# stone-d-chen/ffvvc

Measured on AMD Instinct MI355X. Metric: decoded frames/sec (4K/8K 10-bit VVC) per GPU, higher is better.
Workload: dtype u16

## Files before the change

ffvvc_amd/csrc/itx.hip:

```cpp
#include <type_traits>
#include "common.hpp"
#include "pk16.hpp"
#include "wave.hpp"
#include "runtime.hpp"
#include "resid_math.hpp"
#include "../../include/vvc_mi355.h"
#include "stage_checks.hpp"

namespace vvc355 {

#define VVC355_TABLE(type, name, count) __device__ static const type d_tab_##name[count]
#include "tables.inc"
#undef VVC355_TABLE
#define VVC355_TABLE(type, name, count) static constexpr type c_##name[count]
#include "tables_small.inc"
#undef VVC355_TABLE
__host__ __device__ constexpr int level_scale_of(int rect, int rem)
{
    return rect ? (rem == 0 ? 57 : rem == 1 ? 64 : rem == 2 ? 72 : rem == 3 ? 80 : rem == 4 ? 90 : 102)
                : (rem == 0 ? 40 : rem == 1 ? 45 : rem == 2 ? 51 : rem == 3 ? 57 : rem == 4 ? 64 : 72);
}
static constexpr unsigned long long kDiag4X = 0x3323213210210100ull, kDiag4Y = 0x3231230123012010ull;
constexpr bool itx_small_tables_match()
{
    for (int r = 0; r < 2; r++)
        for (int q = 0; q < 6; q++)
            if (level_scale_of(r, q) != c_level_scale[r * 6 + q]) return false;
    for (int i = 0; i < 16; i++)
        if ((int)((kDiag4X >> (4 * i)) & 15) != c_diag_scan_4x4_x[i] || (int)((kDiag4Y >> (4 * i)) & 15) != c_diag_scan_4x4_y[i]) return false;
    return true;
}
static_assert(itx_small_tables_match(), "level scale / 4x4 diagonal scan differ from vvc_intra.c:329-336 / vvc_data.c:27,152");

enum { TX_DCT2 = 0, TX_DST7 = 1, TX_DCT8 = 2 };

__device__ __forceinline__ const int8_t *dxt_matrix(int type, int n)
{
    if (type == TX_DST7)
        return n == 4 ? d_tab_dst7_4 : n == 8 ? d_tab_dst7_8 : n == 16 ? d_tab_dst7_16 : d_tab_dst7_32;
    return n == 4 ? d_tab_dct8_4 : n == 8 ? d_tab_dct8_8 : n == 16 ? d_tab_dct8_16 : d_tab_dct8_32;
}

__device__ __forceinline__ int inputs_used(int type, int n, int nz)
{
    if (type != TX_DCT2)
        return nz;
    int used = 2;
    while (used < nz)
        used <<= 1;
    used = min(used, n);
    return n == 64 ? min(used, 32) : used;
}

__device__ __forceinline__ int inv_tx_out(int type, int n, int i, const int *in, int step, int cnt, const int8_t *cos_lds)
{
    unsigned acc = 0;
    if (type == TX_DCT2) {
        const int ang = (2 * i + 1) * (64 / n);
        for (int k = 0; k < cnt; k++)
            acc += (unsigned)in[k * step] * (unsigned)(int)cos_lds[(ang * k) & 255];
    } else {
        const int8_t *m = dxt_matrix(type, n) + i;
        for (int k = 0; k < cnt; k++)
            acc += (unsigned)in[k * step] * (unsigned)(int)m[k * n];
    }
    return (int)acc;
}

__host__ __device__ inline int derive_tr_type(int flags, int mts_idx, int lfnst_idx, int c_idx, int w, int h)
{
    const bool isp = flags & VVC355_TU_ISP, sbt = flags & VVC355_TU_SBT;
    if (c_idx || (isp && lfnst_idx))
        return 0;
    bool implicit = false;
    if (flags & VVC355_TU_MTS_ENABLED)
        implicit = isp || (sbt && (w > h ? w : h) <= 32) ||
                   (!(flags & VVC355_TU_EXPLICIT_MTS_INTRA) && (flags & VVC355_TU_INTRA) && !lfnst_idx && !(flags & VVC355_TU_MIP));
    if (implicit) {
        int trh, trv;
        if (sbt) {
            const bool hor = flags & VVC355_TU_SBT_HORIZONTAL, pos = flags & VVC355_TU_SBT_POS;
            trh = (hor || pos) ? 1 : 2;
            trv = (!hor || pos) ? 1 : 2;
        } else {
            trh = (w >= 4 && w <= 16) ? 1 : 0;
            trv = (h >= 4 && h <= 16) ? 1 : 0;
        }
        return trh | (trv << 4);
    }
    const int trh = mts_idx == 0 ? 0 : (mts_idx & 1) ? 1 : 2, trv = mts_idx == 0 ? 0 : mts_idx <= 2 ? 1 : 2;
    return trh | (trv << 4);
}
__device__ __forceinline__ void resolve_type(vvc355_itx_job &job)
{
    if (job.mts_flags & VVC355_ITX_DERIVE_TYPE) {
        const int t = derive_tr_type(job.tu_flags, job.mts_idx, job.lfnst_idx, job.c_idx, 1 << job.log2_w, 1 << job.log2_h);
        job.trh = (uint8_t)(t & 15);
        job.trv = (uint8_t)(t >> 4);
    }
}

struct Dequant {
    int on, scale, bd_shift, bd_offset, range, lw, lh, lm, dc;
    const uint8_t *sm;
    __device__ __forceinline__ void setup(int enable, int lw_, int lh_, int qp_in, int ts, int dep_quant, int bit_depth, int range_,
                                          const uint8_t *sm_, int lm_, int dc_)
    {
        on = enable; lw = lw_; lh = lh_; range = range_; sm = sm_; lm = lm_; dc = dc_;
        const int log_sum = lw + lh, rect = ts ? 0 : (log_sum & 1);
        bd_shift = ts ? 10 : bit_depth + rect + (log_sum / 2) + 10 - range + dep_quant;
        bd_offset = (1 << bd_shift) >> 1;
        const int qp = qp_in + (dep_quant && !ts ? 1 : 0), rem = qp % 6;
        scale = level_scale_of(rect, rem) << (qp / 6);
    }
    __device__ __forceinline__ int apply(int c, int x, int y) const
    {
        if (!on || !c)
            return c;
        int m = 16;
        if (sm) {
            m = gld<uint8_t>(sm + (((y << lm) >> lh) << lm) + ((x << lm) >> lw));
            if (dc >= 0 && x == 0 && y == 0)
                m = dc;
        }
        return clip_intp2((int)((unsigned)c * (unsigned)scale * (unsigned)m + (unsigned)bd_offset) >> bd_shift, range);
    }
    __device__ __forceinline__ int apply_small(int c, int x, int y) const
    {
        if (!on || !c)
            return c;
        int m = 16;
        if (sm) {
            m = gld<uint8_t>(sm + (((y << lm) >> lh) << lm) + ((x << lm) >> lw));
            if (dc >= 0 && x == 0 && y == 0)
                m = dc;
        }
        return clip_intp2((int)((unsigned)__mul24(__mul24(c, m), scale) + (unsigned)bd_offset) >> bd_shift, range);
    }
};

__device__ __forceinline__ Dequant itx_job_dequant(const vvc355_itx_job &job, int bd)
{
    Dequant dq;
    dq.setup(job.dq_flags & 1, job.log2_w, job.log2_h, job.dq_qp, 0, (job.dq_flags >> 1) & 1, bd, job.range,
             (const uint8_t *)job.scale_matrix, job.log2_matrix_size, job.dc);
    return dq;
}

struct LvSrc {
    const vvc355_tb_levels *lv;
    const int16_t *levels;
};
__device__ __forceinline__ LvSrc lv_src() { return LvSrc{ nullptr, nullptr }; }
__device__ __forceinline__ LvSrc lv_src(LvSrc s) { return s; }
__device__ __forceinline__ const int16_t *lv_group(const vvc355_tb_levels &r, const int16_t *levels, int log2_w, int x, int y)
{
    if (x >= 32 || y >= 32)
        return nullptr;
    const int b = (y >> 2) * (((1 << min(log2_w, 5)) + 3) >> 2) + (x >> 2);
    if (!((r.groups >> b) & 1))
        return nullptr;
    return levels + ((size_t)r.first + __popcll(r.groups & ((1ull << b) - 1))) * 16;
}
__device__ __forceinline__ int lv_level(const vvc355_tb_levels &r, const int16_t *levels, int log2_w, int x, int y)
{
    const int16_t *g = lv_group(r, levels, log2_w, x, y);
    return g ? (int)gld<int16_t>(g + (y & 3) * 4 + (x & 3)) : 0;
}
__device__ __forceinline__ int4 unpack_i16x4(uint2 u)
{
    return make_int4((int)(int16_t)(u.x & 0xffff), (int)u.x >> 16, (int)(int16_t)(u.y & 0xffff), (int)u.y >> 16);
}
__device__ __forceinline__ int4 lv_load4(const vvc355_tb_levels &r, const int16_t *levels, int log2_w, int e)
{
    const int w = 1 << log2_w;
    if (w >= 4) {
        const int x = e & (w - 1), y = e >> log2_w;
        const int16_t *g = lv_group(r, levels, log2_w, x, y);
        return g ? unpack_i16x4(gld<uint2>(g + (y & 3) * 4)) : make_int4(0, 0, 0, 0);
    }
    int v[4];
#pragma unroll
    for (int q = 0; q < 4; q++)
        v[q] = lv_level(r, levels, log2_w, (e + q) & (w - 1), (e + q) >> log2_w);
    return make_int4(v[0], v[1], v[2], v[3]);
}

template <int BD, int NT, int CAP, bool PACKED = false, bool LFNST = false, class EPI = void>
__device__ __forceinline__ void itx_generic_block(const vvc355_itx_job &job, int *buf, int *tmp, const int8_t *cos_lds, int tid,
                                                  const vvc355_tb_levels *lvr = nullptr, const int16_t *levels = nullptr,
                                                  int lf_idx = 0, int lf_mode = 0, EPI *epi = nullptr)
{
    constexpr bool WAVE = NT <= 64;
    const int w = 1 << job.log2_w, h = 1 << job.log2_h, n = w * h;
    int nzw = job.nzw, nzh = job.nzh;
    const int range = job.range, bd = job.bd ? job.bd : BD;
    int *coeffs = (int *)job.coeffs;

    constexpr int PER = CAP >= NT ? CAP / NT : 1;
    using px_t = typename Px<BD>::type;
    uint8_t *dst = (uint8_t *)job.dst;
    const int e0 = tid * PER;
    const bool row_io = PER > 1 && w >= PER;
    px_t pred[PER];
    if (dst && e0 < n) {
        if (row_io) {
            const VVC355_GLOBAL px_t *prow = (const VVC355_GLOBAL px_t *)(dst + (ptrdiff_t)(e0 >> job.log2_w) * job.dst_stride) + (e0 & (w - 1));
#pragma unroll
            for (int q = 0; q < PER; q++)
                pred[q] = prow[q];
        } else {
#pragma unroll
            for (int q = 0; q < PER; q++) {
                const int o = e0 + q;
                pred[q] = o < n ? (px_t)ld_px<BD>(dst + (ptrdiff_t)(o >> job.log2_w) * job.dst_stride, o & (w - 1)) : (px_t)0;
            }
        }
    }
    const Dequant dq = itx_job_dequant(job, bd);
    const bool packed = PACKED && !(lvr->flags & VVC355_LEVELS_INT32);
    if (PER < 4) {
#pragma unroll
        for (int q = 0; q < PER; q++)
            if (e0 + q < n) {
                const int x = (e0 + q) & (w - 1), y = (e0 + q) >> job.log2_w;
                buf[e0 + q] = dq.apply(packed ? lv_level(*lvr, levels, job.log2_w, x, y) : gld<int>(coeffs + e0 + q), x, y);
            }
    } else {
#pragma unroll
        for (int c4 = 0; c4 < PER / 4; c4++) {
            const int e = e0 + c4 * 4;
            if (e < n) {
                int4 v = packed ? lv_load4(*lvr, levels, job.log2_w, e) : gld<int4>(coeffs + e);
                if (dq.on) {
                    const int y = e >> job.log2_w, x = e & (w - 1);
                    v.x = dq.apply(v.x, x, y); v.y = dq.apply(v.y, x + 1, y); v.z = dq.apply(v.z, x + 2, y); v.w = dq.apply(v.w, x + 3, y);
                }
                *(int4 *)&buf[e] = v;
            }
        }
    }
    group_sync<NT>();

    if constexpr (LFNST) {
        if (lf_idx) {
            constexpr int MAXO = NT >= 64 ? 1 : NT == 16 ? 3 : 4;
            const bool big = w >= 8 && h >= 8;
            const int n_out = big ? 48 : 16;
            const int nz = ((w == 8 && h == 8) || (w == 4 && h == 4)) ? 8 : 16;
            const int set = lf_mode < 0 ? 1 : d_tab_lfnst_tr_set_index[lf_mode];
            const int8_t *m = big ? d_tab_lfnst_8x8 + (set * 2 + lf_idx - 1) * 16 * 48 : d_tab_lfnst_4x4 + (set * 2 + lf_idx - 1) * 16 * 16;
            unsigned t[MAXO];
#pragma unroll
            for (int q = 0; q < MAXO; q++)
                t[q] = 0;
            for (int i = 0; i < nz; i++) {
                const unsigned u = (unsigned)buf[w * (int)((kDiag4Y >> (4 * i)) & 15) + (int)((kDiag4X >> (4 * i)) & 15)];
#pragma unroll
                for (int q = 0; q < MAXO; q++) {
                    const int j = tid + q * NT;
                    if (j < n_out)
                        t[q] += u * (unsigned)(int)m[i * n_out + j];
                }
            }
            group_sync<NT>();
#pragma unroll
            for (int q = 0; q < MAXO; q++) {
                const int j = tid + q * NT;
                if (j < n_out) {
                    int x, y;
                    if (lf_mode > 34) {
                        if (!big)        { y = j & 3; x = j >> 2; }
                        else if (j < 32) { y = j & 7; x = j >> 3; }
                        else             { y = (j - 32) & 3; x = 4 + ((j - 32) >> 2); }
                    } else {
                        if (!big)        { y = j >> 2; x = j & 3; }
                        else if (j < 32) { y = j >> 3; x = j & 7; }
                        else             { y = 4 + ((j - 32) >> 2); x = (j - 32) & 3; }
                    }
                    buf[y * w + x] = clip_intp2(((int)t[q] + 64) >> 7, range);
                }
            }
            nzw = nzh = big ? 8 : 4;
            group_sync<NT>();
        }
    }

    const bool dc_only = job.trh == TX_DCT2 && job.trv == TX_DCT2 && nzw == 1 && nzh == 1;
    int sh_final;
    if (w > 1 && h > 1) {
        const int sh1 = 7;
        sh_final = 5 + range - bd;
        if (w == h && dc_only) {
            const int t = (buf[0] * 64 + (1 << (sh1 - 1))) >> sh1;
            const int dc = (t * 64 + (1 << (sh_final - 1))) >> sh_final;
            group_sync<NT>();
            for (int i = tid; i < n; i += NT)
                buf[i] = dc;
            sh_final = -1;
        } else if (w >= 4 && h >= 4) {
            const int cnt = inputs_used(job.trv, h, nzh);
            const int cnt2 = inputs_used(job.trh, w, nzw);
            bool small = true;
            for (int i = tid; i < n; i += NT)
                small &= (unsigned)(buf[i] + (1 << 23)) < (1u << 24);
            bool fast1;
            if (WAVE) {
                const unsigned long long gm = (NT == 64 ? ~0ull : ((1ull << (NT & 63)) - 1)) << ((threadIdx.x & 63) & ~(NT - 1));
                fast1 = (__ballot(small) & gm) == gm;
            } else {
                fast1 = (bool)__syncthreads_and(small);
            }
            const int gx = (cnt2 + 3) >> 2, lgh = job.log2_h;
            const int8_t *mv = job.trv == TX_DCT2 ? nullptr : dxt_matrix(job.trv, h);
            for (int g = tid; g < (gx << lgh); g += NT) {
                const int y = g & (h - 1), x0 = (g >> lgh) << 2;
                int acc[4] = { 0, 0, 0, 0 };
                if (x0 < nzw) {
                    const int ang = (2 * y + 1) * (64 >> lgh);
                    int a = 0;
                    for (int k = 0; k < cnt; k++) {
                        const int m = mv ? (int)mv[k * h + y] : (int)cos_lds[a];
                        a = (a + ang) & 255;
                        const int4 v = *(const int4 *)&buf[k * w + x0];
                        if (fast1) {
                            acc[0] += __mul24(m, v.x); acc[1] += __mul24(m, v.y); acc[2] += __mul24(m, v.z); acc[3] += __mul24(m, v.w);
                        } else {
                            acc[0] += m * v.x; acc[1] += m * v.y; acc[2] += m * v.z; acc[3] += m * v.w;
                        }
                    }
                }
#pragma unroll
                for (int q = 0; q < 4; q++) {
                    const int x = x0 + q;
                    if (x < w)
                        tmp[x * h + y] = x < nzw ? clip_intp2((acc[q] + (1 << (sh1 - 1))) >> sh1, range) : 0;
                }
            }
            group_sync<NT>();
            const int8_t *mh = job.trh == TX_DCT2 ? nullptr : dxt_matrix(job.trh, w);
            for (int g = tid; g < (n >> 2); g += NT) {
                const int x = g & (w - 1), y0 = (g >> job.log2_w) << 2;
                const int ang = (2 * x + 1) * (64 >> job.log2_w);
                int acc[4] = { 0, 0, 0, 0 }, a = 0;
                for (int k = 0; k < cnt2; k++) {
                    const int m = mh ? (int)mh[k * w + x] : (int)cos_lds[a];
                    a = (a + ang) & 255;
                    const int4 v = *(const int4 *)&tmp[k * h + y0];
                    acc[0] += __mul24(m, v.x); acc[1] += __mul24(m, v.y); acc[2] += __mul24(m, v.z); acc[3] += __mul24(m, v.w);
                }
#pragma unroll
                for (int q = 0; q < 4; q++)
                    buf[(y0 + q) * w + x] = acc[q];
            }
        } else {
            const int cnt = inputs_used(job.trv, h, nzh);
            for (int o = tid; o < n; o += NT) {
                const int y = o >> job.log2_w, x = o & (w - 1);
                int v = 0;
                if (x < nzw) {
                    v = inv_tx_out(job.trv, h, y, buf + x, w, cnt, cos_lds);
                    v = clip_intp2((v + (1 << (sh1 - 1))) >> sh1, range);
                }
                tmp[o] = v;
            }
            group_sync<NT>();
            const int cnt2 = inputs_used(job.trh, w, nzw);
            for (int o = tid; o < n; o += NT) {
                const int y = o >> job.log2_w, x = o & (w - 1);
                buf[o] = inv_tx_out(job.trh, w, x, tmp + y * w, 1, cnt2, cos_lds);
            }
        }
    } else {
        sh_final = 6 + range - bd;
        if (dc_only) {
            const int dc = (buf[0] * 64 + (1 << (sh_final - 1))) >> sh_final;
            group_sync<NT>();
            for (int i = tid; i < n; i += NT)
                buf[i] = dc;
            sh_final = -1;
        } else {
            const int type = w > 1 ? job.trh : job.trv, nz = w > 1 ? nzw : nzh;
            const int cnt = inputs_used(type, n, nz);
            for (int o = tid; o < n; o += NT)
                tmp[o] = inv_tx_out(type, n, o, buf, 1, cnt, cos_lds);
            group_sync<NT>();
            for (int o = tid; o < n; o += NT)
                buf[o] = tmp[o];
        }
    }
    group_sync<NT>();
    if (e0 < n) {
        int r[PER];
#pragma unroll
        for (int q = 0; q < PER; q++) {
            const int o = e0 + q;
            r[q] = o < n ? (sh_final < 0 ? buf[o] : (buf[o] + (1 << (sh_final - 1))) >> sh_final) : 0;
        }
        if constexpr (!std::is_void<EPI>::value) {
#pragma unroll
            for (int q = 0; q < PER; q++)
                if (e0 + q < n)
                    epi->sample((e0 + q) & (w - 1), (e0 + q) >> job.log2_w, e0 + q, r[q]);
            return;
        }
        if (job.store_coeffs) {
            if (PER < 4) {
#pragma unroll
                for (int q = 0; q < PER; q++)
                    if (e0 + q < n)
                        gst<int>(coeffs + e0 + q, r[q]);
            } else {
#pragma unroll
                for (int c4 = 0; c4 < PER / 4; c4++)
                    if (e0 + c4 * 4 < n)
                        gst<int4>(coeffs + e0 + c4 * 4, make_int4(r[c4 * 4], r[c4 * 4 + 1], r[c4 * 4 + 2], r[c4 * 4 + 3]));
            }
        }
        if (dst) {
            if (row_io) {
                VVC355_GLOBAL px_t *prow = (VVC355_GLOBAL px_t *)(dst + (ptrdiff_t)(e0 >> job.log2_w) * job.dst_stride) + (e0 & (w - 1));
                px_t outv[PER];
#pragma unroll
                for (int q = 0; q < PER; q++)
                    outv[q] = (px_t)clip_px<BD>((int)pred[q] + r[q]);
#pragma unroll
                for (int q = 0; q < PER; q++)
                    prow[q] = outv[q];
            } else {
#pragma unroll
                for (int q = 0; q < PER; q++) {
                    const int o = e0 + q;
                    if (o < n)
                        st_px<BD>(dst + (ptrdiff_t)(o >> job.log2_w) * job.dst_stride, o & (w - 1), clip_px<BD>((int)pred[q] + r[q]));
                }
            }
        }
    }
}

template <int BD, int NT, int CAP, typename... Lv>
__global__ __launch_bounds__(256) void itx_kernel(const vvc355_itx_job *__restrict__ jobs, int n_jobs, Lv... lv)
{
    constexpr bool PACKED = sizeof...(Lv) > 0;
    constexpr int TBS = 256 / NT;
    __shared__ __attribute__((aligned(16))) int buf_all[TBS][CAP];
    __shared__ __attribute__((aligned(16))) int tmp_all[TBS][CAP];
    __shared__ int8_t cos_lds[256];
    cos_lds[threadIdx.x] = d_tab_dct2_cos[threadIdx.x];
    __syncthreads();
    const int sub = threadIdx.x / NT, tid = threadIdx.x % NT;
    const int ji = blockIdx.x * TBS + sub;
    if (ji >= n_jobs)
        return;
    vvc355_itx_job job = jobs[ji];
    resolve_type(job);
    if (job.log2_w + job.log2_h > __builtin_ctz(CAP))
        return;
    if constexpr (PACKED) {
        const LvSrc ls = lv_src(lv...);
        const vvc355_tb_levels r = ls.lv[ji];
        itx_generic_block<BD, NT, CAP, true>(job, buf_all[sub], tmp_all[sub], cos_lds, tid, &r, ls.levels);
    } else {
        itx_generic_block<BD, NT, CAP>(job, buf_all[sub], tmp_all[sub], cos_lds, tid);
    }
}


template <int N> struct TxDim {
    static constexpr int KV = N < 32 ? N : 32;
    static constexpr int P = KV + (KV >= 16 ? 8 : 0);
    static constexpr int KS = KV < 8 ? 4 : 8;
    static constexpr int NTYPE = N <= 32 ? 3 : 1;
    __device__ static __forceinline__ const int16_t *table()
    {
        return N == 4 ? d_tab_itx16_4 : N == 8 ? d_tab_itx16_8 : N == 16 ? d_tab_itx16_16 : N == 32 ? d_tab_itx16_32 : d_tab_itx16_64;
    }
    __device__ static __forceinline__ void stage(int16_t *lds)
    {
        const int16_t *src = table();
        constexpr int ND = NTYPE * N * KV / 2;
        for (int i = threadIdx.x; i < ND; i += 256) {
            const int row = i / (KV / 2), c2 = i % (KV / 2);
            *(uint32_t *)&lds[row * P + 2 * c2] = gld<uint32_t>(src + 2 * i);
        }
    }
};

template <int KS> __device__ __forceinline__ void lds_row(const int16_t *p, uint32_t (&d)[KS / 2])
{
    if constexpr (KS == 8) {
        const uint4 v = *(const uint4 *)p;
        d[0] = v.x; d[1] = v.y; d[2] = v.z; d[3] = v.w;
    } else {
        const uint2 v = *(const uint2 *)p;
        d[0] = v.x; d[1] = v.y;
    }
}

template <int BD> __device__ __forceinline__ uint2 px4_load(const uint8_t *p)
{
    uint2 v = make_uint2(0, 0);
    if (BD > 8) v = gld<uint2>(p);
    else v.x = gld<uint32_t>(p);
    return v;
}
template <int BD> __device__ __forceinline__ void px4_add_store(uint8_t *p, uint2 praw, const int (&res)[4])
{
    if (BD > 8) {
        const int o0 = clip_px<BD>((int)(praw.x & 0xffff) + res[0]), o1 = clip_px<BD>((int)(praw.x >> 16) + res[1]);
        const int o2 = clip_px<BD>((int)(praw.y & 0xffff) + res[2]), o3 = clip_px<BD>((int)(praw.y >> 16) + res[3]);
        gst<uint2>(p, make_uint2((uint32_t)o0 | ((uint32_t)o1 << 16), (uint32_t)o2 | ((uint32_t)o3 << 16)));
    } else {
        const uint32_t pr = praw.x;
        const int o0 = clip_px<BD>((int)(pr & 0xff) + res[0]), o1 = clip_px<BD>((int)((pr >> 8) & 0xff) + res[1]);
        const int o2 = clip_px<BD>((int)((pr >> 16) & 0xff) + res[2]), o3 = clip_px<BD>((int)(pr >> 24) + res[3]);
        gst<uint32_t>(p, (uint32_t)o0 | ((uint32_t)o1 << 8) | ((uint32_t)o2 << 16) | ((uint32_t)o3 << 24));
    }
}

template <int BD, int LW, int LH, typename... Lv>
__global__ __launch_bounds__(256) void itx_shape_kernel(const vvc355_itx_job *__restrict__ jobs, int n_jobs, Lv... lv)
{
    constexpr bool PACKED = sizeof...(Lv) > 0;
#include "itx_shape_body.inc"
}

__global__ __launch_bounds__(256) void levels_expand_kernel(const vvc355_itx_job *__restrict__ jobs, LvSrc ls, int n_jobs)
{
    const int ji = blockIdx.x * 4 + (threadIdx.x >> 6), lane = threadIdx.x & 63;
    if (ji >= n_jobs)
        return;
    const vvc355_tb_levels r = ls.lv[ji];
    if (r.flags & VVC355_LEVELS_INT32)
        return;
    const vvc355_itx_job job = jobs[ji];
    int *coeffs = (int *)job.coeffs;
    const int lw = job.log2_w, w = 1 << lw;
    const int nzw = min((int)job.nzw, w), nzh = min((int)job.nzh, 1 << job.log2_h);
    const int sw = (nzw + 3) >> 2;
    for (int u = lane; u < sw * nzh; u += 64) {
        const int y = u / sw, x0 = (u - y * sw) * 4;
        const int16_t *g = lv_group(r, ls.levels, lw, x0, y);
        const int4 v = g ? unpack_i16x4(gld<uint2>(g + (y & 3) * 4)) : make_int4(0, 0, 0, 0);
        int *row = coeffs + y * w + x0;
        gst<int>(row, v.x);
        if (x0 + 1 < nzw) gst<int>(row + 1, v.y);
// ... 172 lines not shown

__global__ __launch_bounds__(256) void itx_build_kernel(const vvc355_itx_frame *__restrict__ fp)
{
    constexpr int WG = 256, JOB_DW = sizeof(vvc355_itx_job) / 4, RES_DW = sizeof(vvc355_lmcs_resid_job) / 4;
    __shared__ uint32_t s_jobs[WG * (JOB_DW + 1)], s_resid[WG * (RES_DW + 1)];
    const vvc355_itx_frame f = load_uniform(fp);
    const int tid = threadIdx.x, first = blockIdx.x * WG, n = min(WG, f.n_tus - first);
    if (tid < n) {
        uint32_t tw[sizeof(vvc355_itx_tu) / 4];
#pragma unroll
        for (int k = 0; k < 4; k++) tw[k] = gld<uint32_t>((const uint32_t *)f.tus + (size_t)(first + tid) * 4 + k);
        vvc355_itx_tu t;
        __builtin_memcpy(&t, tw, sizeof(t));
        vvc355_itx_job j = {};
        j.coeffs = f.coeffs + (uint64_t)t.coeff_off * 4;
        const int c = t.c_idx;
        const uint64_t plane = c == 0 ? f.plane[0] : c == 1 ? f.plane[1] : f.plane[2];
        const int stride = c == 0 ? f.stride[0] : c == 1 ? f.stride[1] : f.stride[2];
        const bool keep = (t.flags & 4) != 0;
        j.dst = keep ? 0 : plane + (uint64_t)t.y0 * stride + ((uint64_t)t.x0 << f.pixel_shift);
        j.dst_stride = stride;
        j.trh = t.tr & 15; j.trv = t.tr >> 4;
        j.log2_w = t.log2_w; j.log2_h = t.log2_h; j.nzw = t.nzw; j.nzh = t.nzh;
        j.range = f.range; j.bd = f.bd;
        j.store_coeffs = keep;
        j.dq_flags = (uint8_t)((t.flags & 1) | (t.flags & 2)); j.dq_qp = t.qp;
        j.log2_matrix_size = 1; j.dc = -1;
        j.mts_flags = (t.flags & 8) ? VVC355_ITX_DERIVE_TYPE : 0; j.tu_flags = f.tu_flags; j.c_idx = t.c_idx;
        lds_row_put<JOB_DW + 1>(s_jobs, tid, j);
        if (f.resid_jobs) {
            vvc355_lmcs_resid_job r = {};
            if (t.flags & 64) {
                r.dst = plane + (uint64_t)t.y0 * stride + ((uint64_t)t.x0 << f.pixel_shift);
                r.resid = j.coeffs; r.luma = f.plane[0];
                r.dst_stride = stride; r.luma_stride = f.stride[0];
                r.w = (int16_t)(1 << t.log2_w); r.h = (int16_t)(1 << t.log2_h);
                r.x_vpdu = (int16_t)((t.x0 << (c ? f.hs : 0)) & ~(f.size_y - 1)); r.y_vpdu = (int16_t)((t.y0 << (c ? f.vs : 0)) & ~(f.size_y - 1));
                r.pic_w = (int16_t)f.width; r.pic_h = (int16_t)f.height; r.size_y = f.size_y;
                r.avail_l = (t.flags >> 4) & 1; r.avail_t = (t.flags >> 5) & 1;
                r.joint = 8;
                if (f.scale_table) {
                    const int ux = (f.width + f.size_y - 1) / f.size_y;
                    r.luma = f.scale_table + (uint64_t)((r.y_vpdu / f.size_y) * ux + r.x_vpdu / f.size_y) * 2;
                    r.joint = 8 | 16;
                }
            }
            lds_row_put<RES_DW + 1>(s_resid, tid, r);
        }
    }
    __syncthreads();
    lds_rows_to_global<JOB_DW, JOB_DW + 1>(s_jobs, (vvc355_itx_job *)f.jobs + first, n);
    if (f.resid_jobs)
        lds_rows_to_global<RES_DW, RES_DW + 1>(s_resid, (vvc355_lmcs_resid_job *)f.resid_jobs + first, n);
}

template <int NT, int CAP, bool PACKED>
__device__ __forceinline__ void intra_tb_group(const vvc355_intra_tb_frame &f, int first, int end, int wg, int *buf, int *tmp,
                                               const int8_t *cos_lds)
{
    constexpr int TBS = 256 / NT;
    const int sub = threadIdx.x / NT, tid = threadIdx.x % NT;
    const int i = first + wg * TBS + sub;
    if (i >= end)
        return;
    const vvc355_intra_tu t = ((const vvc355_intra_tu *)f.tus)[i];
    const int lw = t.log2_w, lh = t.log2_h;
    const bool lfnst = t.flags & VVC355_INTRA_TU_LFNST;
    if (lw + lh > __builtin_ctz(CAP) || lw + lh < 2 || lw > 6 || lh > 6 || (t.flags & ~(VVC355_INTRA_TU_DEP_QUANT | VVC355_INTRA_TU_LFNST)))
        return;
    if (lfnst && (lw < 2 || lh < 2 || t.lfnst_idx < 1 || t.lfnst_idx > 2 || t.pred_mode_intra > 94))
        return;
    vvc355_itx_job job = {};
    job.coeffs = f.coeffs + (uint64_t)t.coeff_off * 4;
    job.log2_w = t.log2_w; job.log2_h = t.log2_h;
    job.nzw = (uint8_t)min((int)t.nzw, 1 << lw); job.nzh = (uint8_t)min((int)t.nzh, 1 << lh);
    job.range = f.range; job.bd = f.bd;
    job.store_coeffs = 1;
    job.dq_flags = (uint8_t)(1 | ((t.flags & VVC355_INTRA_TU_DEP_QUANT) << 1)); job.dq_qp = t.qp;
    job.log2_matrix_size = 1; job.dc = -1;
    job.mts_flags = VVC355_ITX_DERIVE_TYPE; job.tu_flags = t.tu_flags; job.mts_idx = t.mts_idx; job.lfnst_idx = t.lfnst_idx; job.c_idx = t.c_idx;
    resolve_type(job);
    if constexpr (PACKED) {
        const vvc355_tb_levels r = ((const vvc355_tb_levels *)f.lv)[i];
        itx_generic_block<10, NT, CAP, true, true>(job, buf + sub * CAP, tmp + sub * CAP, cos_lds, tid, &r, (const int16_t *)f.levels,
                                                   lfnst ? t.lfnst_idx : 0, t.pred_mode_intra);
    } else {
        itx_generic_block<10, NT, CAP, false, true>(job, buf + sub * CAP, tmp + sub * CAP, cos_lds, tid, nullptr, nullptr,
                                                    lfnst ? t.lfnst_idx : 0, t.pred_mode_intra);
    }
}

template <int NT, int CAP, bool PACKED>
__global__ __launch_bounds__(256) void intra_tb_kernel(const vvc355_intra_tb_frame *__restrict__ fp, int first, int end)
{
    constexpr int TBS = 256 / NT;
    __shared__ __attribute__((aligned(16))) int buf_all[TBS * CAP];
    __shared__ __attribute__((aligned(16))) int tmp_all[TBS * CAP];
    __shared__ int8_t cos_lds[256];
    cos_lds[threadIdx.x] = d_tab_dct2_cos[threadIdx.x];
    __syncthreads();
    const vvc355_intra_tb_frame f = load_uniform(fp);
    intra_tb_group<NT, CAP, PACKED>(f, first, end, blockIdx.x, buf_all, tmp_all, cos_lds);
}

struct IntraTbGrid {
    int wg_first[4];
};
template <bool PACKED>
__global__ __launch_bounds__(256) void intra_tb_merged_kernel(const vvc355_intra_tb_frame *__restrict__ fp, IntraTbGrid g)
{
    __shared__ __attribute__((aligned(16))) int buf_all[1024];
    __shared__ __attribute__((aligned(16))) int tmp_all[1024];
    __shared__ int8_t cos_lds[256];
    cos_lds[threadIdx.x] = d_tab_dct2_cos[threadIdx.x];
    __syncthreads();
    const vvc355_intra_tb_frame f = load_uniform(fp);
    const int b = blockIdx.x;
    if (b < g.wg_first[0])
        intra_tb_group<4, 16, PACKED>(f, f.class_first[0], f.class_first[1], b, buf_all, tmp_all, cos_lds);
    else if (b < g.wg_first[1])
        intra_tb_group<16, 64, PACKED>(f, f.class_first[1], f.class_first[2], b - g.wg_first[0], buf_all, tmp_all, cos_lds);
    else if (b < g.wg_first[2])
        intra_tb_group<64, 256, PACKED>(f, f.class_first[2], f.class_first[3], b - g.wg_first[1], buf_all, tmp_all, cos_lds);
    else if (b < g.wg_first[3])
        intra_tb_group<256, 1024, PACKED>(f, f.class_first[3], f.class_first[4], b - g.wg_first[2], buf_all, tmp_all, cos_lds);
}

static constexpr int kIntraTbDefaultMode = 2;

template <bool PACKED>
static void launch_intra_tb(hipStream_t st, const vvc355_intra_tb_frame *fd, const vvc355_intra_tb_frame &fh, int mode)
{
    const int32_t *cf = fh.class_first;
    int wgs[5];
    for (int k = 0; k < 5; k++) {
        const int cnt = cf[k + 1] - cf[k], tbs = k == 0 ? 64 : k == 1 ? 16 : k == 2 ? 4 : 1;
        wgs[k] = (cnt + tbs - 1) / tbs;
    }
    if (mode == 2) {
        IntraTbGrid g;
        int total = 0;
        for (int k = 0; k < 4; k++)
            g.wg_first[k] = total += wgs[k];
        if (total)
            hipLaunchKernelGGL((intra_tb_merged_kernel<PACKED>), dim3(total), dim3(256), 0, st, fd, g);
    } else {
        if (wgs[0]) hipLaunchKernelGGL((intra_tb_kernel<4, 16, PACKED>), dim3(wgs[0]), dim3(256), 0, st, fd, cf[0], cf[1]);
        if (wgs[1]) hipLaunchKernelGGL((intra_tb_kernel<16, 64, PACKED>), dim3(wgs[1]), dim3(256), 0, st, fd, cf[1], cf[2]);
        if (wgs[2]) hipLaunchKernelGGL((intra_tb_kernel<64, 256, PACKED>), dim3(wgs[2]), dim3(256), 0, st, fd, cf[2], cf[3]);
        if (wgs[3]) hipLaunchKernelGGL((intra_tb_kernel<256, 1024, PACKED>), dim3(wgs[3]), dim3(256), 0, st, fd, cf[3], cf[4]);
    }
    if (wgs[4]) hipLaunchKernelGGL((intra_tb_kernel<256, 4096, PACKED>), dim3(wgs[4]), dim3(256), 0, st, fd, cf[4], cf[5]);
}

template <int BD> struct InterEpi {
    uint8_t *dst0, *dst1;
    int stride0, stride1;
    int *keep;
    int joint, scale;
    uint2 p0[4], p1[4];
    static constexpr int PXS = (int)sizeof(typename Px<BD>::type);
    __device__ __forceinline__ void prefetch(bool act, int x0, int y0)
    {
#pragma unroll
        for (int r = 0; r < 4; r++) {
            p0[r] = p1[r] = make_uint2(0, 0);
            if (act && !keep) {
                p0[r] = px4_load<BD>(dst0 + row_off(y0 + r, stride0) + x0 * PXS);
                if (dst1)
                    p1[r] = px4_load<BD>(dst1 + row_off(y0 + r, stride1) + x0 * PXS);
            }
        }
    }
    template <int W> __device__ __forceinline__ void row(int r, int x0, int y, const int (&res)[4])
    {
        if (keep) {
            gst<int4>(keep + y * W + x0, make_int4(res[0], res[1], res[2], res[3]));
            return;
        }
        int own[4], other[4];
#pragma unroll
        for (int q = 0; q < 4; q++) {
            own[q] = resid_sample<BD>(res[q], joint & 8, scale);
            other[q] = resid_sample<BD>(res[q], joint, scale);
        }
        px4_add_store<BD>(dst0 + row_off(y, stride0) + x0 * PXS, p0[r], own);
        if (dst1)
            px4_add_store<BD>(dst1 + row_off(y, stride1) + x0 * PXS, p1[r], other);
    }
    __device__ __forceinline__ void sample(int x, int y, int o, int r)
    {
        if (keep) {
            gst<int>(keep + o, r);
            return;
        }
        uint8_t *row0 = dst0 + row_off(y, stride0);
        st_px<BD>(row0, x, clip_px<BD>(ld_px<BD>(row0, x) + resid_sample<BD>(r, joint & 8, scale)));
// ... 22 lines not shown
            return vvc355_tb_levels{ 0, 0, VVC355_LEVELS_INT32 };
        const uint4 v = gld<uint4>((const vvc355_tb_levels *)f.lv + first + i);
        return vvc355_tb_levels{ (uint64_t)v.x | ((uint64_t)v.y << 32), v.z, v.w };
    }
    __device__ __forceinline__ const int16_t *stream() const { return (const int16_t *)f.levels; }
    __device__ __forceinline__ bool get(int i, vvc355_itx_job &job, Epi &epi) const
    {
        vvc355_inter_tu t;
        const uint4 raw = gld<uint4>((const vvc355_inter_tu *)f.tus + first + i);
        __builtin_memcpy(&t, &raw, sizeof(t));
        const int lw = t.log2_w, lh = t.log2_h, c = t.flags & 3, joint = t.joint_mts & 15, mts = (t.joint_mts >> 4) & 7;
        const bool keep = t.flags & VVC355_INTER_TU_KEEP;
        bool ok = lw <= 6 && lh <= 6 && lw + lh >= 2 && ((lw >= 2 && lh >= 2) ? (lw - 2) * 5 + (lh - 2) : 25) == bin;
        ok &= !(t.flags & 0xc0) && !(t.joint_mts & 0x80) && mts <= 4 && c != 3 && (c != 0) == (ch != 0) && !(c == 0 && joint);
        ok &= !((joint & 8) && !f.scale_table);
        const int hs = c ? f.hs : 0, vs = c ? f.vs : 0;
        ok &= t.x0 >= 0 && t.y0 >= 0 && t.x0 + (1 << (lw & 7)) <= (f.width >> hs) && t.y0 + (1 << (lh & 7)) <= (f.height >> vs);
        if (keep || (levels_of(i).flags & VVC355_LEVELS_INT32))
            ok &= !(t.coeff_off & 3);
        int scale = 0;
        if (ok && (joint & 8)) {
            const int ls = f.size_y == 64 ? 6 : 5;
            const int ux = ((t.x0 << hs) >> ls) - ((t.flags >> 4) & 1), uy = ((t.y0 << vs) >> ls) - ((t.flags >> 5) & 1);
            ok = ux >= 0 && uy >= 0;
            if (ok)
                scale = (int)gld<int16_t>((const int16_t *)f.scale_table + uy * ((f.width + (1 << ls) - 1) >> ls) + ux);
        }
        job = {};
        job.log2_w = (uint8_t)(ok ? lw : lw0); job.log2_h = (uint8_t)(ok ? lh : lh0);
        job.nzw = job.nzh = 1;
        job.range = f.range; job.bd = f.bd;
        job.log2_matrix_size = 1; job.dc = -1;
        epi.dst0 = epi.dst1 = nullptr;
        epi.keep = nullptr;
        epi.stride0 = epi.stride1 = 0;
        epi.joint = epi.scale = 0;
        if (!ok)
            return false;
        job.coeffs = f.coeffs + (uint64_t)t.coeff_off * 4;
        job.nzw = (uint8_t)min((int)t.nzw, 1 << lw); job.nzh = (uint8_t)min((int)t.nzh, 1 << lh);
        job.dq_flags = (uint8_t)(1 | ((t.flags & VVC355_INTER_TU_DEP_QUANT) ? 2 : 0)); job.dq_qp = t.qp;
        job.mts_flags = VVC355_ITX_DERIVE_TYPE; job.tu_flags = t.tu_flags; job.mts_idx = (uint8_t)mts; job.c_idx = (uint8_t)c;
        resolve_type(job);
        if (((lw < 2 || lw > 5) && job.trh) || ((lh < 2 || lh > 5) && job.trv)) {
            job.trh = job.trv = 0;
            return false;
        }
        const uint64_t p0 = f.plane[0], p1 = f.plane[1], p2 = f.plane[2];
        const int s0 = f.stride[0], s1 = f.stride[1], s2 = f.stride[2];
        const uint64_t plane = c == 0 ? p0 : c == 1 ? p1 : p2, other = c == 1 ? p2 : p1;
        const int stride = c == 0 ? s0 : c == 1 ? s1 : s2, ostride = c == 1 ? s2 : s1;
        if (keep) {
            epi.keep = (int *)job.coeffs;
            return true;
        }
        epi.dst0 = (uint8_t *)plane + row_off(t.y0, stride) + t.x0 * Epi::PXS;
        epi.stride0 = stride;
        if (joint & 1) {
            epi.dst1 = (uint8_t *)other + row_off(t.y0, ostride) + t.x0 * Epi::PXS;
            epi.stride1 = ostride;
        }
        epi.joint = joint;
        epi.scale = scale;
        return true;
    }
};

template <int BD, int LW, int LH>
__global__ __launch_bounds__(256) void inter_tb_shape_kernel(const vvc355_inter_tb_frame *__restrict__ fp, int first, int end, int ch)
{
    constexpr bool PACKED = true;
    const InterTbSrc<BD> src{ load_uniform((const InterTbHead *)fp), first, ch, (LW - 2) * 5 + (LH - 2), LW, LH };
    const int n_jobs = end - first;
#define ITX_SHAPE_RECORDS
#include "itx_shape_body.inc"
#undef ITX_SHAPE_RECORDS
}

template <int BD>
__global__ __launch_bounds__(256) void inter_tb_thin_kernel(const vvc355_inter_tb_frame *__restrict__ fp, int first, int end, int ch)
{
    __shared__ __attribute__((aligned(16))) int buf_all[4 * 256];
    __shared__ __attribute__((aligned(16))) int tmp_all[4 * 256];
    __shared__ int8_t cos_lds[256];
    cos_lds[threadIdx.x] = d_tab_dct2_cos[threadIdx.x];
    __syncthreads();
    const int sub = threadIdx.x >> 6, tid = threadIdx.x & 63;
    const int i = xcd_chunked(blockIdx.x, gridDim.x) * 4 + sub;
    if (i >= end - first)
        return;
    const InterTbSrc<BD> src{ load_uniform((const InterTbHead *)fp), first, ch, 25, 1, 1 };
    vvc355_itx_job job;
    InterEpi<BD> epi;
    if (!src.get(i, job, epi))
        return;
    const vvc355_tb_levels r = src.levels_of(i);
    itx_generic_block<BD, 64, 256, true, false, InterEpi<BD>>(job, buf_all + sub * 256, tmp_all + sub * 256, cos_lds, tid, &r, src.stream(), 0, 0, &epi);
}

template <int BD, int LW>
static void launch_inter_tb_shape(hipStream_t st, const vvc355_inter_tb_frame *fd, int first, int end, int ch, int log2_h)
{
#define VVC355_INTER_TB_SHAPE(LH)                                                                                     \
    case LH: {                                                                                                        \
        constexpr int TBS = 256 / ((1 << (LW + LH)) / 16);                                                            \
        hipLaunchKernelGGL((inter_tb_shape_kernel<BD, LW, LH>), dim3((end - first + TBS - 1) / TBS), dim3(256), 0, st, fd, first, end, ch); \
    } break;
    switch (log2_h) {
    VVC355_INTER_TB_SHAPE(2) VVC355_INTER_TB_SHAPE(3) VVC355_INTER_TB_SHAPE(4) VVC355_INTER_TB_SHAPE(5) VVC355_INTER_TB_SHAPE(6)
    }
#undef VVC355_INTER_TB_SHAPE
}

template <int BD>
static void launch_inter_tb(hipStream_t st, const vvc355_inter_tb_frame *fd, const vvc355_inter_tb_frame &fh, int channels)
{
    for (int ch = 0; ch < 2; ch++) {
        if (!(channels & (1 << ch)))
            continue;
        for (int bin = 0; bin < VVC355_INTER_TB_BINS; bin++) {
            const int first = fh.bin_first[ch][bin], end = fh.bin_first[ch][bin + 1];
            if (end <= first)
                continue;
            if (bin == 25) {
                hipLaunchKernelGGL((inter_tb_thin_kernel<BD>), dim3((end - first + 3) / 4), dim3(256), 0, st, fd, first, end, ch);
                continue;
            }
            switch (bin / 5 + 2) {
            case 2: launch_inter_tb_shape<BD, 2>(st, fd, first, end, ch, bin % 5 + 2); break;
            case 3: launch_inter_tb_shape<BD, 3>(st, fd, first, end, ch, bin % 5 + 2); break;
            case 4: launch_inter_tb_shape<BD, 4>(st, fd, first, end, ch, bin % 5 + 2); break;
            case 5: launch_inter_tb_shape<BD, 5>(st, fd, first, end, ch, bin % 5 + 2); break;
            case 6: launch_inter_tb_shape<BD, 6>(st, fd, first, end, ch, bin % 5 + 2); break;
            }
        }
    }
}


struct TsTbHead {
    uint64_t tus, coeffs, lv, levels, plane[3], scale_table;
    int32_t  stride[3], width, height, n_tus;
    uint8_t  hs, vs, size_y, range, bd, pad_[3];
};
static_assert(sizeof(TsTbHead) == offsetof(vvc355_ts_tb_frame, class_first) && offsetof(TsTbHead, hs) == offsetof(vvc355_ts_tb_frame, hs) &&
              offsetof(TsTbHead, stride) == offsetof(vvc355_ts_tb_frame, stride), "TsTbHead is the frame without class_first");

struct TsTbGrid {
    int wg_first[4];
    int first[5];
};

template <int MAXP>
__device__ __forceinline__ void ts_bdpcm_lines(int (&v)[4][4], int pos, int stride, int range)
{
    const int lane = threadIdx.x & 63;
    int s[4], lo[4], hi[4], out[4], cin[4];
#pragma unroll
    for (int l = 0; l < 4; l++) {
        s[l] = out[l] = v[l][0];
        lo[l] = -(1 << range); hi[l] = (1 << range) - 1;
        cin[l] = 0;
#pragma unroll
        for (int k = 1; k < 4; k++) {
            s[l] += v[l][k];
            lo[l] = clip_intp2(lo[l] + v[l][k], range); hi[l] = clip_intp2(hi[l] + v[l][k], range);
            out[l] = clip_intp2(out[l] + v[l][k], range);
        }
    }
#pragma unroll
    for (int p = 1; p < MAXP; p++) {
#pragma unroll
        for (int l = 0; l < 4; l++) {
            const int prev = __shfl(out[l], lane - stride);
            if (pos == p) {
                cin[l] = prev;
                out[l] = clip3(prev + s[l], lo[l], hi[l]);
            }
        }
    }
// ... 519 lines not shown
```

Baseline: 631.8.

## Stage DST7/DCT8 matrices in LDS and fetch only nonzero coefficient window

New measurement: 633.9, median of 6. No clear change (+0.3%).

```diff
diff --git a/ffvvc_amd/csrc/itx.hip b/ffvvc_amd/csrc/itx.hip
--- a/ffvvc_amd/csrc/itx.hip
+++ b/ffvvc_amd/csrc/itx.hip
@@ -9,7 +9,7 @@
 
 namespace vvc355 {
 
-#define VVC355_TABLE(type, name, count) __device__ static const type d_tab_##name[count]
+#define VVC355_TABLE(type, name, count) __device__ static const __attribute__((aligned(16))) type d_tab_##name[count]
 #include "tables.inc"
 #undef VVC355_TABLE
 #define VVC355_TABLE(type, name, count) static constexpr type c_##name[count]
@@ -39,6 +39,35 @@
     if (type == TX_DST7)
         return n == 4 ? d_tab_dst7_4 : n == 8 ? d_tab_dst7_8 : n == 16 ? d_tab_dst7_16 : d_tab_dst7_32;
     return n == 4 ? d_tab_dct8_4 : n == 8 ? d_tab_dct8_8 : n == 16 ? d_tab_dct8_16 : d_tab_dct8_32;
+}
+
+#ifndef VVC355_ITX_GENERIC_LEVERS
+#define VVC355_ITX_GENERIC_LEVERS 3
+#endif
+static constexpr bool kItxWindowFetch = (VVC355_ITX_GENERIC_LEVERS & 1) != 0, kItxLdsMatrices = (VVC355_ITX_GENERIC_LEVERS & 2) != 0;
+
+struct TxLds {
+    static constexpr int kCos = 256, kPerType = 16 + 64 + 256 + 1024;
+    static constexpr int kBytes = kCos + (kItxLdsMatrices ? 2 * kPerType : 0);
+    __device__ static __forceinline__ int off(int type, int n)
+    {
+        return kCos + (type - 1) * kPerType + (n == 4 ? 0 : n == 8 ? 16 : n == 16 ? 16 + 64 : 16 + 64 + 256);
+    }
+};
+template <int N> __device__ __forceinline__ void tx_lds_copy(int8_t *lds, const int8_t *tab)
+{
+    for (int i = threadIdx.x; i < N / 4; i += 256)
+        ((uint32_t *)lds)[i] = ((const uint32_t *)tab)[i];
+}
+__device__ __forceinline__ void tx_lds_stage(int8_t *lds)
+{
+    tx_lds_copy<256>(lds, d_tab_dct2_cos);
+    if (kItxLdsMatrices) {
+        tx_lds_copy<16>(lds + TxLds::off(TX_DST7, 4), d_tab_dst7_4);       tx_lds_copy<16>(lds + TxLds::off(TX_DCT8, 4), d_tab_dct8_4);
+        tx_lds_copy<64>(lds + TxLds::off(TX_DST7, 8), d_tab_dst7_8);       tx_lds_copy<64>(lds + TxLds::off(TX_DCT8, 8), d_tab_dct8_8);
+        tx_lds_copy<256>(lds + TxLds::off(TX_DST7, 16), d_tab_dst7_16);    tx_lds_copy<256>(lds + TxLds::off(TX_DCT8, 16), d_tab_dct8_16);
+        tx_lds_copy<1024>(lds + TxLds::off(TX_DST7, 32), d_tab_dst7_32);   tx_lds_copy<1024>(lds + TxLds::off(TX_DCT8, 32), d_tab_dct8_32);
+    }
 }
 
 __device__ __forceinline__ int inputs_used(int type, int n, int nz)
@@ -52,6 +81,7 @@
     return n == 64 ? min(used, 32) : used;
 }
 
+template <bool LTAB = false>
 __device__ __forceinline__ int inv_tx_out(int type, int n, int i, const int *in, int step, int cnt, const int8_t *cos_lds)
 {
     unsigned acc = 0;
@@ -59,6 +89,10 @@
         const int ang = (2 * i + 1) * (64 / n);
         for (int k = 0; k < cnt; k++)
             acc += (unsigned)in[k * step] * (unsigned)(int)cos_lds[(ang * k) & 255];
+    } else if (LTAB) {
+        const int8_t *m = cos_lds + TxLds::off(type, n) + i;
+        for (int k = 0; k < cnt; k++)
+            acc += (unsigned)in[k * step] * (unsigned)(int)m[k * n];
     } else {
         const int8_t *m = dxt_matrix(type, n) + i;
         for (int k = 0; k < cnt; k++)
@@ -186,7 +220,7 @@
     return make_int4(v[0], v[1], v[2], v[3]);
 }
 
-template <int BD, int NT, int CAP, bool PACKED = false, bool LFNST = false, class EPI = void>
+template <int BD, int NT, int CAP, bool PACKED = false, bool LFNST = false, class EPI = void, bool LTAB = false>
 __device__ __forceinline__ void itx_generic_block(const vvc355_itx_job &job, int *buf, int *tmp, const int8_t *cos_lds, int tid,
                                                   const vvc355_tb_levels *lvr = nullptr, const int16_t *levels = nullptr,
                                                   int lf_idx = 0, int lf_mode = 0, EPI *epi = nullptr)
@@ -219,28 +253,65 @@
     }
     const Dequant dq = itx_job_dequant(job, bd);
     const bool packed = PACKED && !(lvr->flags & VVC355_LEVELS_INT32);
+    int frows = h, fcols = w;
+    if (kItxWindowFetch) {
+        const bool dc0 = job.trh == TX_DCT2 && job.trv == TX_DCT2 && nzw == 1 && nzh == 1;
+        if (LFNST && lf_idx)
+            frows = fcols = (w >= 8 && h >= 8) ? 8 : 4;
+        else if (w > 1 && h > 1) {
+            frows = (dc0 && w == h) ? 1 : inputs_used(job.trv, h, nzh);
+            fcols = (dc0 && w == h) ? 1 : nzw;
+        } else if (w > 1) {
+            frows = 1;
+            fcols = dc0 ? 1 : inputs_used(job.trh, n, nzw);
+        } else {
+            fcols = 1;
+            frows = dc0 ? 1 : inputs_used(job.trv, n, nzh);
+        }
+    }
+    bool small = true;
     if (PER < 4) {
 #pragma unroll
         for (int q = 0; q < PER; q++)
             if (e0 + q < n) {
                 const int x = (e0 + q) & (w - 1), y = (e0 + q) >> job.log2_w;
-                buf[e0 + q] = dq.apply(packed ? lv_level(*lvr, levels, job.log2_w, x, y) : gld<int>(coeffs + e0 + q), x, y);
+                int v = 0;
+                if (y < frows && x < fcols)
+                    v = dq.apply(packed ? lv_level(*lvr, levels, job.log2_w, x, y) : gld<int>(coeffs + e0 + q), x, y);
+                small &= (unsigned)(v + (1 << 23)) < (1u << 24);
+                buf[e0 + q] = v;
             }
     } else {
 #pragma unroll
         for (int c4 = 0; c4 < PER / 4; c4++) {
             const int e = e0 + c4 * 4;
             if (e < n) {
-                int4 v = packed ? lv_load4(*lvr, levels, job.log2_w, e) : gld<int4>(coeffs + e);
-                if (dq.on) {
-                    const int y = e >> job.log2_w, x = e & (w - 1);
-                    v.x = dq.apply(v.x, x, y); v.y = dq.apply(v.y, x + 1, y); v.z = dq.apply(v.z, x + 2, y); v.w = dq.apply(v.w, x + 3, y);
+                const int y = e >> job.log2_w, x = e & (w - 1);
+                int4 v = make_int4(0, 0, 0, 0);
+                if (y < frows && x < fcols) {
+                    v = packed ? lv_load4(*lvr, levels, job.log2_w, e) : gld<int4>(coeffs + e);
+                    if (dq.on) {
+                        v.x = dq.apply(v.x, x, y); v.y = dq.apply(v.y, x + 1, y); v.z = dq.apply(v.z, x + 2, y); v.w = dq.apply(v.w, x + 3, y);
+                    }
+                    small &= (unsigned)(v.x + (1 << 23)) < (1u << 24) && (unsigned)(v.y + (1 << 23)) < (1u << 24) &&
+                             (unsigned)(v.z + (1 << 23)) < (1u << 24) && (unsigned)(v.w + (1 << 23)) < (1u << 24);
                 }
                 *(int4 *)&buf[e] = v;
             }
         }
     }
-    group_sync<NT>();
+    bool fast1 = true;
+    if (kItxWindowFetch) {
+        if (WAVE) {
+            wave_sync();
+            const unsigned long long gm = (NT == 64 ? ~0ull : ((1ull << (NT & 63)) - 1)) << ((threadIdx.x & 63) & ~(NT - 1));
+            fast1 = (__ballot(small) & gm) == gm;
+        } else {
+            fast1 = (bool)__syncthreads_and(small);
+        }
+    } else {
+        group_sync<NT>();
+    }
 
     if constexpr (LFNST) {
         if (lf_idx) {
@@ -301,27 +372,30 @@
         } else if (w >= 4 && h >= 4) {
             const int cnt = inputs_used(job.trv, h, nzh);
             const int cnt2 = inputs_used(job.trh, w, nzw);
-            bool small = true;
-            for (int i = tid; i < n; i += NT)
-                small &= (unsigned)(buf[i] + (1 << 23)) < (1u << 24);
-            bool fast1;
-            if (WAVE) {
-                const unsigned long long gm = (NT == 64 ? ~0ull : ((1ull << (NT & 63)) - 1)) << ((threadIdx.x & 63) & ~(NT - 1));
-                fast1 = (__ballot(small) & gm) == gm;
-            } else {
-                fast1 = (bool)__syncthreads_and(small);
+            if (!kItxWindowFetch) {
+                bool sm = true;
+                for (int i = tid; i < n; i += NT)
+                    sm &= (unsigned)(buf[i] + (1 << 23)) < (1u << 24);
+                if (WAVE) {
+                    const unsigned long long gm = (NT == 64 ? ~0ull : ((1ull << (NT & 63)) - 1)) << ((threadIdx.x & 63) & ~(NT - 1));
+                    fast1 = (__ballot(sm) & gm) == gm;
+                } else {
+                    fast1 = (bool)__syncthreads_and(sm);
+                }
             }
             const int gx = (cnt2 + 3) >> 2, lgh = job.log2_h;
-            const int8_t *mv = job.trv == TX_DCT2 ? nullptr : dxt_matrix(job.trv, h);
+            const int8_t *mv = job.trv == TX_DCT2 ? nullptr : LTAB ? nullptr : dxt_matrix(job.trv, h);
+            const int8_t *mv_lds = cos_lds + (LTAB && job.trv != TX_DCT2 ? TxLds::off(job.trv, h) : 0);
+            const bool mv_dxt = job.trv != TX_DCT2;
             for (int g = tid; g < (gx << lgh); g += NT) {
                 const int y = g & (h - 1), x0 = (g >> lgh) << 2;
                 int acc[4] = { 0, 0, 0, 0 };
                 if (x0 < nzw) {
-                    const int ang = (2 * y + 1) * (64 >> lgh);
-                    int a = 0;
+                    const int ang = LTAB && mv_dxt ? h : (2 * y + 1) * (64 >> lgh), amask = LTAB && mv_dxt ? ~0 : 255;
+                    int a = LTAB && mv_dxt ? y : 0;
                     for (int k = 0; k < cnt; k++) {
-                        const int m = mv ? (int)mv[k * h + y] : (int)cos_lds[a];
-                        a = (a + ang) & 255;
+                        const int m = mv ? (int)mv[k * h + y] : (int)mv_lds[a];
+                        a = (a + ang) & amask;
                         const int4 v = *(const int4 *)&buf[k * w + x0];
                         if (fast1) {
                             acc[0] += __mul24(m, v.x); acc[1] += __mul24(m, v.y); acc[2] += __mul24(m, v.z); acc[3] += __mul24(m, v.w);
@@ -338,14 +412,16 @@
                 }
             }
             group_sync<NT>();
-            const int8_t *mh = job.trh == TX_DCT2 ? nullptr : dxt_matrix(job.trh, w);
+            const int8_t *mh = job.trh == TX_DCT2 ? nullptr : LTAB ? nullptr : dxt_matrix(job.trh, w);
+            const int8_t *mh_lds = cos_lds + (LTAB && job.trh != TX_DCT2 ? TxLds::off(job.trh, w) : 0);
+            const bool mh_dxt = job.trh != TX_DCT2;
             for (int g = tid; g < (n >> 2); g += NT) {
                 const int x = g & (w - 1), y0 = (g >> job.log2_w) << 2;
-                const int ang = (2 * x + 1) * (64 >> job.log2_w);
-                int acc[4] = { 0, 0, 0, 0 }, a = 0;
+                const int ang = LTAB && mh_dxt ? w : (2 * x + 1) * (64 >> job.log2_w), amask = LTAB && mh_dxt ? ~0 : 255;
+                int acc[4] = { 0, 0, 0, 0 }, a = LTAB && mh_dxt ? x : 0;
                 for (int k = 0; k < cnt2; k++) {
-                    const int m = mh ? (int)mh[k * w + x] : (int)cos_lds[a];
-                    a = (a + ang) & 255;
+                    const int m = mh ? (int)mh[k * w + x] : (int)mh_lds[a];
+                    a = (a + ang) & amask;
                     const int4 v = *(const int4 *)&tmp[k * h + y0];
                     acc[0] += __mul24(m, v.x); acc[1] += __mul24(m, v.y); acc[2] += __mul24(m, v.z); acc[3] += __mul24(m, v.w);
                 }
@@ -359,7 +435,7 @@
                 const int y = o >> job.log2_w, x = o & (w - 1);
                 int v = 0;
                 if (x < nzw) {
-                    v = inv_tx_out(job.trv, h, y, buf + x, w, cnt, cos_lds);
+                    v = inv_tx_out<LTAB>(job.trv, h, y, buf + x, w, cnt, cos_lds);
                     v = clip_intp2((v + (1 << (sh1 - 1))) >> sh1, range);
                 }
                 tmp[o] = v;
@@ -368,7 +444,7 @@
             const int cnt2 = inputs_used(job.trh, w, nzw);
             for (int o = tid; o < n; o += NT) {
                 const int y = o >> job.log2_w, x = o & (w - 1);
-                buf[o] = inv_tx_out(job.trh, w, x, tmp + y * w, 1, cnt2, cos_lds);
+                buf[o] = inv_tx_out<LTAB>(job.trh, w, x, tmp + y * w, 1, cnt2, cos_lds);
             }
         }
     } else {
@@ -383,7 +459,7 @@
             const int type = w > 1 ? job.trh : job.trv, nz = w > 1 ? nzw : nzh;
             const int cnt = inputs_used(type, n, nz);
             for (int o = tid; o < n; o += NT)
-                tmp[o] = inv_tx_out(type, n, o, buf, 1, cnt, cos_lds);
+                tmp[o] = inv_tx_out<LTAB>(type, n, o, buf, 1, cnt, cos_lds);
             group_sync<NT>();
             for (int o = tid; o < n; o += NT)
                 buf[o] = tmp[o];
@@ -446,23 +522,23 @@
     constexpr int TBS = 256 / NT;
     __shared__ __attribute__((aligned(16))) int buf_all[TBS][CAP];
     __shared__ __attribute__((aligned(16))) int tmp_all[TBS][CAP];
-    __shared__ int8_t cos_lds[256];
-    cos_lds[threadIdx.x] = d_tab_dct2_cos[threadIdx.x];
-    __syncthreads();
+    __shared__ __attribute__((aligned(16))) int8_t cos_lds[TxLds::kBytes];
     const int sub = threadIdx.x / NT, tid = threadIdx.x % NT;
     const int ji = blockIdx.x * TBS + sub;
+    vvc355_itx_job job = jobs[min(ji, n_jobs - 1)];
+    tx_lds_stage(cos_lds);
+    __syncthreads();
     if (ji >= n_jobs)
         return;
-    vvc355_itx_job job = jobs[ji];
     resolve_type(job);
     if (job.log2_w + job.log2_h > __builtin_ctz(CAP))
         return;
     if constexpr (PACKED) {
         const LvSrc ls = lv_src(lv...);
         const vvc355_tb_levels r = ls.lv[ji];
-        itx_generic_block<BD, NT, CAP, true>(job, buf_all[sub], tmp_all[sub], cos_lds, tid, &r, ls.levels);
+        itx_generic_block<BD, NT, CAP, true, false, void, kItxLdsMatrices>(job, buf_all[sub], tmp_all[sub], cos_lds, tid, &r, ls.levels);
     } else {
-        itx_generic_block<BD, NT, CAP>(job, buf_all[sub], tmp_all[sub], cos_lds, tid);
+        itx_generic_block<BD, NT, CAP, false, false, void, kItxLdsMatrices>(job, buf_all[sub], tmp_all[sub], cos_lds, tid);
     }
 }
 
@@ -801,10 +877,10 @@
     resolve_type(job);
     if constexpr (PACKED) {
         const vvc355_tb_levels r = ((const vvc355_tb_levels *)f.lv)[i];
-        itx_generic_block<10, NT, CAP, true, true>(job, buf + sub * CAP, tmp + sub * CAP, cos_lds, tid, &r, (const int16_t *)f.levels,
+        itx_generic_block<10, NT, CAP, true, true, void, kItxLdsMatrices>(job, buf + sub * CAP, tmp + sub * CAP, cos_lds, tid, &r, (const int16_t *)f.levels,
                                                    lfnst ? t.lfnst_idx : 0, t.pred_mode_intra);
     } else {
-        itx_generic_block<10, NT, CAP, false, true>(job, buf + sub * CAP, tmp + sub * CAP, cos_lds, tid, nullptr, nullptr,
+        itx_generic_block<10, NT, CAP, false, true, void, kItxLdsMatrices>(job, buf + sub * CAP, tmp + sub * CAP, cos_lds, tid, nullptr, nullptr,
                                                     lfnst ? t.lfnst_idx : 0, t.pred_mode_intra);
     }
 }
@@ -815,8 +891,8 @@
     constexpr int TBS = 256 / NT;
     __shared__ __attribute__((aligned(16))) int buf_all[TBS * CAP];
     __shared__ __attribute__((aligned(16))) int tmp_all[TBS * CAP];
-    __shared__ int8_t cos_lds[256];
-    cos_lds[threadIdx.x] = d_tab_dct2_cos[threadIdx.x];
+    __shared__ __attribute__((aligned(16))) int8_t cos_lds[TxLds::kBytes];
+    tx_lds_stage(cos_lds);
     __syncthreads();
     const vvc355_intra_tb_frame f = load_uniform(fp);
     intra_tb_group<NT, CAP, PACKED>(f, first, end, blockIdx.x, buf_all, tmp_all, cos_lds);
@@ -830,8 +906,8 @@
 {
     __shared__ __attribute__((aligned(16))) int buf_all[1024];
     __shared__ __attribute__((aligned(16))) int tmp_all[1024];
-    __shared__ int8_t cos_lds[256];
-    cos_lds[threadIdx.x] = d_tab_dct2_cos[threadIdx.x];
+    __shared__ __attribute__((aligned(16))) int8_t cos_lds[TxLds::kBytes];
+    tx_lds_stage(cos_lds);
     __syncthreads();
     const vvc355_intra_tb_frame f = load_uniform(fp);
     const int b = blockIdx.x;
@@ -1020,8 +1096,8 @@
 {
     __shared__ __attribute__((aligned(16))) int buf_all[4 * 256];
     __shared__ __attribute__((aligned(16))) int tmp_all[4 * 256];
-    __shared__ int8_t cos_lds[256];
-    cos_lds[threadIdx.x] = d_tab_dct2_cos[threadIdx.x];
+    __shared__ __attribute__((aligned(16))) int8_t cos_lds[TxLds::kBytes];
+    tx_lds_stage(cos_lds);
     __syncthreads();
     const int sub = threadIdx.x >> 6, tid = threadIdx.x & 63;
     const int i = xcd_chunked(blockIdx.x, gridDim.x) * 4 + sub;
@@ -1033,7 +1109,7 @@
     if (!src.get(i, job, epi))
         return;
     const vvc355_tb_levels r = src.levels_of(i);
-    itx_generic_block<BD, 64, 256, true, false, InterEpi<BD>>(job, buf_all + sub * 256, tmp_all + sub * 256, cos_lds, tid, &r, src.stream(), 0, 0, &epi);
+    itx_generic_block<BD, 64, 256, true, false, InterEpi<BD>, kItxLdsMatrices>(job, buf_all + sub * 256, tmp_all + sub * 256, cos_lds, tid, &r, src.stream(), 0, 0, &epi);
 }
 
 template <int BD, int LW>
```
